# sandialabs/tenzing

Measured on AMD Instinct MI355X. Metric: best-schedule iter time (ms) + MCTS search wall-clock, 3D halo-exchange 8 ranks, lower is better.
Workload: dtype fp64

## Files before the change

### tenzing_amd/csrc/bind/module.cpp

```cpp
#include <pybind11/functional.h>
#include <pybind11/numpy.h>
#include <pybind11/pybind11.h>
#include <pybind11/stl.h>

#include "core/benchmark.hpp"
#include "core/health.hpp"
#include "core/solve.hpp"
#include "hip/comm_ops.hpp"
#include "hip/hip_runtime.hpp"
#include "hip/rccl_comm.hpp"
#include "hip/rocsparse_spmv.hpp"
#include "kernels/kernels.hpp"
#include "workloads/workloads.hpp"

#include <hip/hip_runtime_api.h>

#include <csignal>
#include <cstdlib>
#include <execinfo.h>
#include <sstream>
#include <unistd.h>
#include <vector>

namespace py = pybind11;
// ... 545 lines not shown
        for (auto &x : in) l.append(py::bytes(x));
        return l;
      }, "personalized exchange: element j goes to rank j; returns what each rank sent me");
  py::class_<SelfCtrl, Ctrl, std::shared_ptr<SelfCtrl>>(m, "SelfCtrl").def(py::init<>());
  py::class_<TcpCtrl, Ctrl, std::shared_ptr<TcpCtrl>>(m, "TcpCtrl")
      .def(py::init<int, int>())
      .def("listen", &TcpCtrl::listen, py::arg("port") = 0, py::arg("bind_addr") = "0.0.0.0")
      .def("connect", &TcpCtrl::connect, py::arg("host"), py::arg("port"), py::arg("timeout_s") = 300.0,
           py::call_guard<py::gil_scoped_release>())
      .def("rendezvous", &TcpCtrl::rendezvous, py::arg("host"), py::arg("port"),
           py::arg("timeout_s") = 300.0, py::arg("nports") = 8, py::call_guard<py::gil_scoped_release>(),
           "rank 0 listens on the first free port of port..port+nports-1, the others connect "
           "(handshake-checked): no store, no torch")
      .def("rendezvous_file", &TcpCtrl::rendezvous_file, py::arg("path"), py::arg("host") = "127.0.0.1",
           py::arg("timeout_s") = 300.0, py::call_guard<py::gil_scoped_release>())
      .def("ensure_timeout", &TcpCtrl::ensure_timeout, py::arg("seconds"),
           "raise the peer sockets' receive timeout to at least this (never lowered)")
      .def_property_readonly("timeout", &TcpCtrl::timeout,
                             "the peer sockets' receive timeout in seconds (0 = none)");
  py::class_<MpiCtrl, Ctrl, std::shared_ptr<MpiCtrl>>(m, "MpiCtrl")
      .def(py::init<const std::string &>(), py::arg("lib") = "", py::call_guard<py::gil_scoped_release>())
      .def_static("launched", &MpiCtrl::launched)
      .def_static("launcher_size", &MpiCtrl::launcher_size)
      .def_static("launcher_local_rank", &MpiCtrl::launcher_local_rank)
      .def_property_readonly("library", &MpiCtrl::library);

  py::class_<MctsOpts>(m, "MctsOpts")
      .def(py::init<>())
      .def_readwrite("n_iters", &MctsOpts::n_iters)
      .def_readwrite("time_budget_s", &MctsOpts::time_budget_s)
      .def_readwrite("max_tree_nodes", &MctsOpts::max_tree_nodes)
      .def_readwrite("seed_schedules", &MctsOpts::seed_schedules)
      .def_readwrite("expand_rollout", &MctsOpts::expand_rollout)
      .def_readwrite("remove_redundant_syncs", &MctsOpts::remove_redundant_syncs)
      .def_readwrite("reuse_measurements", &MctsOpts::reuse_measurements)
      .def_readwrite("verify", &MctsOpts::verify)
      .def_readwrite("dump_tree", &MctsOpts::dump_tree)
      .def_readwrite("dump_tree_prefix", &MctsOpts::dump_tree_prefix)
      .def_readwrite("strategy", &MctsOpts::strategy)
      .def_readwrite("seed", &MctsOpts::seed)
      .def_readwrite("explore_c", &MctsOpts::explore_c)
      .def_readwrite("bench", &MctsOpts::bench)
      .def_readwrite("checkpoint_path", &MctsOpts::checkpoint_path)
      .def_readwrite("checkpoint_every", &MctsOpts::checkpoint_every)
      .def_readwrite("resume_path", &MctsOpts::resume_path)
      .def_readwrite("trap_signals", &MctsOpts::trap_signals)
      .def_readwrite("skip_failed", &MctsOpts::skip_failed)
      .def("json", [](const MctsOpts &o) { return o.json().dump(); });
  py::class_<DfsOpts>(m, "DfsOpts")
      .def(py::init<>())
      .def_readwrite("max_seqs", &DfsOpts::max_seqs)
      .def_readwrite("dedup_states", &DfsOpts::dedup_states)
      .def_readwrite("remove_redundant_syncs", &DfsOpts::remove_redundant_syncs)
      .def_readwrite("bench", &DfsOpts::bench)
      .def_readwrite("trap_signals", &DfsOpts::trap_signals)
      .def_readwrite("skip_failed", &DfsOpts::skip_failed)
      .def("json", [](const DfsOpts &o) { return o.json().dump(); });
  py::class_<SimResult>(m, "SimResult")
      .def_readonly("seq", &SimResult::seq)
      .def_readonly("res", &SimResult::res)
      .def_readonly("cached", &SimResult::cached)
      .def_readonly("seeded", &SimResult::seeded);
  py::class_<SearchResult>(m, "SearchResult")
      .def_readonly("sims", &SearchResult::sims)
      .def_readonly("wall_s", &SearchResult::wall_s)
      .def_readonly("tree_size", &SearchResult::tree_size)
      .def_readonly("tree_fully_visited", &SearchResult::tree_fully_visited)
      .def_readonly("stop_reason", &SearchResult::stop_reason)
      .def_readonly("failed", &SearchResult::failed)
      .def_readonly("dead_domains", &SearchResult::dead_domains)
      .def_readonly("pruned_dead", &SearchResult::pruned_dead)
      .def("best", &SearchResult::best)
      .def("counters", [](const SearchResult &r) { return counters_dict(r.counters); })
      .def("counter_counts", [](const SearchResult &r) {
        py::dict d;
        for (const auto &kv : r.counters.counts) d[py::str(kv.first)] = kv.second;
        return d;
      }, "how often each counter was hit (phases; SEED_IN_TREE: seeds placed in the tree)")
      .def("dump_csv", [](const SearchResult &r) {
        std::ostringstream ss;
        r.dump_csv(ss);
        return ss.str();
      })
      .def("dump_jsonl", [](const SearchResult &r) {
        std::ostringstream ss;
        r.dump_jsonl(ss);
        return ss.str();
      });
  py::class_<RunDeadline>(m, "RunDeadline")
      .def(py::init<double, int>(), py::arg("seconds"), py::arg("exit_code") = 5)
      .def("set_report", &RunDeadline::set_report, py::arg("line"))
      .def("cancel", &RunDeadline::cancel)
      .def("tighten", &RunDeadline::tighten, py::arg("seconds"), py::arg("exit_code"),
           "expire at the latest `seconds` from now, exiting with `exit_code`")
      .def_property_readonly("remaining", &RunDeadline::remaining)
      .def_property_readonly("armed", &RunDeadline::armed);
  m.def("exit_with_report", [](int code, const std::string &why) { exit_with_report(code, why); },
        py::arg("code"), py::arg("why"),
        "leave the process now (no cleanup), printing the armed RunDeadline's report line with "
        "\"exit_reason\" added: what the watchdog does when a hung run cannot be released");
  m.def("mcts_explore", [](std::shared_ptr<Graph> g, const Platform &p, Benchmarker &b, Ctrl &c,
                           const MctsOpts &o, py::object cb) {
    std::function<void(size_t, const SimResult &)> f;
    if (!cb.is_none()) {
// ... 437 lines not shown
  py::class_<DistSpmv, std::shared_ptr<DistSpmv>>(m, "DistSpmv")
      .def(py::init([](const SpmvArgs &a, Ctrl *c) {
             py::gil_scoped_release r;
             return std::make_shared<DistSpmv>(a, c);
           }), py::arg("args"), py::arg("ctrl") = nullptr)
      .def_property_readonly("args", &DistSpmv::args)
      .def("local_rows", &DistSpmv::local_rows)
      .def("local_nnz", &DistSpmv::local_nnz)
      .def("remote_nnz", &DistSpmv::remote_nnz)
      .def("remote_cols", &DistSpmv::remote_cols)
      .def("send_elems", &DistSpmv::send_elems)
      .def("num_peers", &DistSpmv::num_peers)
      .def("transport", &DistSpmv::transport)
      .def("uses_ipc", &DistSpmv::uses_ipc)
      .def("uses_rccl", &DistSpmv::uses_rccl)
      .def("rccl_graph_ok", &DistSpmv::rccl_graph_ok, "RCCL exchanges may be captured into hipGraphs")
      .def("rccl_capture_note", &DistSpmv::rccl_capture_note,
           "how the RCCL exchange is compiled into hipGraphs (its preflight's verdict), or why not")
      .def("ipc_errors", &DistSpmv::ipc_errors, py::call_guard<py::gil_scoped_release>())
      .def("setup", [](DistSpmv &s, Ctrl *c) { s.setup(c); }, py::arg("ctrl") = nullptr,
           py::call_guard<py::gil_scoped_release>())
      .def("ready", &DistSpmv::ready)
      .def("add_to_graph", &DistSpmv::add_to_graph)
      .def("op_graph", [](DistSpmv &s) { return std::const_pointer_cast<Graph>(s.op_graph()); })
      .def("check", [](DistSpmv &s, uintptr_t st) { return s.check(P(st)); }, py::arg("stream") = 0)
      .def("reset_y", [](DistSpmv &s, uintptr_t st) { s.reset_y(P(st)); }, py::arg("stream") = 0);
  m.def("move_spmv_op", [](std::shared_ptr<HaloExchange> h, std::vector<int> dirs, std::shared_ptr<DistSpmv> s,
                           std::string name, int lanes, bool intoY) {
    return make_move_spmv_op(h, std::move(dirs), s, std::move(name), lanes, intoY);
  }, py::arg("halo"), py::arg("dirs"), py::arg("spmv"), py::arg("name"), py::arg("lanes") = kern::kSpmvIlp + 4,
     py::arg("into_y") = true,
     "one GPU op running the halo's self moves `dirs` and the SpMV's local product in one kernel "
     "(horizontal fusion; the SpMV's workgroups interleaved among the move's)");
  m.def("random_band_matrix", [](int64_t n, int64_t bw, int64_t nnz, uint64_t seed) {
    CsrHost a = random_band_matrix(n, bw, nnz, seed);
    return py::make_tuple(a.rowPtr, a.colInd, a.val);
  });
  m.def("spd_band_matrix", [](int64_t n, int64_t bw, int64_t nnz, uint64_t seed) {
    CsrHost a = spd_band_matrix(n, bw, nnz, seed);
    return py::make_tuple(a.rowPtr, a.colInd, a.val);
  }, py::arg("n"), py::arg("bw"), py::arg("nnz"), py::arg("seed"),
     "symmetric, strictly diagonally dominant band matrix (mirrored random_band_matrix off-diagonals, "
     "a_ii = 1 + sum |a_ij|) as (rowPtr, colInd, val)");
  py::class_<CgArgs>(m, "CgArgs")
      .def(py::init<>())
      .def_readwrite("m", &CgArgs::m)
      .def_readwrite("bw", &CgArgs::bw)
      .def_readwrite("nnz", &CgArgs::nnz)
      .def_readonly("nnz_actual", &CgArgs::nnz_actual)
      .def_readwrite("seed", &CgArgs::seed)
      .def_readwrite("matrix", &CgArgs::matrix)
      .def_readwrite("device", &CgArgs::device)
      .def_readwrite("form", &CgArgs::form)
      .def_readwrite("lanes", &CgArgs::lanes)
      .def_readwrite("rhs", &CgArgs::rhs)
      .def_readwrite("nrhs", &CgArgs::nrhs)
      .def_readwrite("rhs_first", &CgArgs::rhs_first)
      .def_readwrite("prefix", &CgArgs::prefix)
      .def_readwrite("rank", &CgArgs::rank)
      .def_readwrite("size", &CgArgs::size)
      .def("json", [](const CgArgs &a) { return a.json().dump(); });
  {
    auto f32 = [](const std::vector<float> &v) { return py::array_t<float>(py::ssize_t(v.size()), v.data()); };
    py::class_<ConjugateGradient, std::shared_ptr<ConjugateGradient>>(m, "ConjugateGradient")
        .def(py::init([](const CgArgs &a) { return std::make_shared<ConjugateGradient>(a); }), py::arg("args"))
        .def_property_readonly("args", &ConjugateGradient::args)
// ... 477 lines not shown
```

### tenzing_amd/csrc/core/solve.cpp

```cpp
#include "solve.hpp"
#include "health.hpp"

#include <algorithm>
#include <chrono>
#include <cmath>
#include <condition_variable>
#include <csignal>
#include <cstdio>
#include <cstring>
#include <unistd.h>

#include <atomic>
#include <fstream>
#include <iostream>
#include <limits>
#include <map>
#include <mutex>
#include <sstream>
#include <thread>
#include <unordered_map>
#include <unordered_set>

#ifndef TZ_VERSION_MAJOR
#define TZ_VERSION_MAJOR 0
// ... 230 lines not shown
  void backprop(MctsNode &node, const BenchResult &br) override { push_sorted(node.times, br.pct10); }
};

}

std::vector<std::string> strategy_names() {
  return {"FastMin", "Coverage", "Random", "AvgTime", "Unvisited", "AntiCorrelation",
          "NormalizedAntiCorrelation", "NormRootCorr", "BalanceHistogram"};
}

std::unique_ptr<Strategy> make_strategy(const std::string &name, uint64_t seed) {
  std::string n = name;
  std::transform(n.begin(), n.end(), n.begin(), ::tolower);
  n.erase(std::remove(n.begin(), n.end(), '_'), n.end());
  if (n == "fastmin" || n == "mintime") return std::make_unique<FastMin>();
  if (n == "coverage") return std::make_unique<Coverage>();
  if (n == "random") return std::make_unique<RandomS>(seed);
  if (n == "avgtime") return std::make_unique<AvgTime>();
  if (n == "unvisited") return std::make_unique<Unvisited>();
  if (n == "anticorrelation" || n == "anticorr") return std::make_unique<AntiCorrelation>();
  if (n == "normalizedanticorrelation" || n == "normanticorr") return std::make_unique<NormCorr>(true);
  if (n == "normrootcorr") return std::make_unique<NormCorr>(false);
  if (n == "balancehistogram" || n == "balancehist") return std::make_unique<BalanceHistogram>();
  TZ_THROW("unknown MCTS strategy '" << name << "'");
}


Json MctsOpts::json() const {
  Json j, o;
  o["nIters"] = n_iters;
  o["timeBudgetS"] = time_budget_s;
  if (max_tree_nodes > 0) o["maxTreeNodes"] = max_tree_nodes;
  o["expandRollout"] = expand_rollout;
  o["removeRedundantSyncs"] = remove_redundant_syncs;
  o["reuseMeasurements"] = reuse_measurements;
  o["strategy"] = strategy;
  o["seed"] = int64_t(seed);
  o["exploreC"] = explore_c;
  o["benchOpts"] = bench.json();
  j["mcts__Opts"] = o;
  return j;
}

namespace {

struct Tree {
  MctsNode root;
  std::unique_ptr<Strategy> strat;
  std::mt19937_64 rng;
  double c;
  size_t nodes = 1;
  std::set<std::string> dead;
  size_t prunedDead = 0;

  bool dead_decision(const State &st, const Decision &d) const {
    if (dead.empty()) return false;
    if (d.kind == Decision::Kind::Choose) {
      const auto alts = static_cast<const ChoiceOp &>(*st.graph().op(d.node)).choices();
      return uses_domain(alts[size_t(d.choice)], dead);
    }
    if (d.kind == Decision::Kind::Execute && d.op) return uses_domain(d.op, dead);
    if (d.kind == Decision::Kind::Assign) return uses_domain(st.graph().op(d.node), dead);
    return false;
  }

  static void propagate_visited(MctsNode *node) {
    for (; node; node = node->parent) {
      if (node->children.empty() || node->fully_visited) continue;
      bool all = true;
      for (auto &ch : node->children) all = all && ch->fully_visited;
      if (!all) break;
      node->fully_visited = true;
    }
  }

  bool prune_dead_children(MctsNode &node, const State &st) {
    bool live = false;
    if (!dead.empty())
      for (auto &ch : node.children)
        if (!ch->fully_visited && dead_decision(st, ch->decision)) {
          ch->fully_visited = true;
          ++prunedDead;
        }
    for (auto &ch : node.children) live = live || !ch->fully_visited;
    if (!node.children.empty() && !live) propagate_visited(&node);
    return live || node.children.empty();
// ... 171 lines not shown
        const Decision &d = ch[i]->decision;
        if (d.kind != Decision::Kind::Execute || d.op->op_class() != OpClass::Sync || d.op->kind() != want.kind())
          continue;
        if (ws < 0 || (m != relabel.end() && m->second == sync_stream(*d.op))) pick = int(i);
      }
      ++pos;
      if (pick < 0) continue;
    }
    if (pick < 0 && pos < seed.size()) {
      for (size_t i = 0; i < ch.size() && pick < 0; ++i) {
        const Decision &d = ch[i]->decision;
        if (d.kind == Decision::Kind::Execute && d.op->op_class() != OpClass::Sync &&
            d.op->name() == seed[pos]->name()) {
          pick = int(i);
          advance = true;
        }
      }
    }
    for (size_t i = 0; i < ch.size() && pick < 0; ++i) {
      const Decision &d = ch[i]->decision;
      if (d.kind == Decision::Kind::Execute && d.op->op_class() == OpClass::Sync) pick = int(i);
    }
    if (pick < 0) return nullptr;
    if (advance) ++pos;
    st.apply_inplace(ch[size_t(pick)]->decision);
    cur = ch[size_t(pick)].get();
  }
  tree.ensure_children(*cur, st);
  Sequence s = st.sequence();
  if (removeRedundant) remove_redundant_syncs(s, st.graph(), nStreams);
  return s.canonical_key() == seed.canonical_key() ? cur : nullptr;
}

void graphviz_rec(const MctsNode &node, const Strategy &strat, std::ostream &os, size_t &count,
                  size_t maxNodes, const std::string &id) {
  std::string color = node.fully_visited ? "green" : "black";
  os << "  " << id << " [label=\"" << node.decision.desc() << "\\nn=" << node.n << "\\n"
     << strat.label(node) << "\", color=" << color << "];\n";
  ++count;
  size_t i = 0;
  for (const auto &ch : node.children) {
    ++i;
    if (count >= maxNodes) break;
    if (ch->n == 0) continue;
    const std::string cid = id + "_" + std::to_string(i);
    if (ch->fully_visited || ch->n == 1) {
      os << "  " << cid << " [label=\"" << ch->decision.desc() << "\\nn=" << ch->n
         << "\", color=" << (ch->fully_visited ? "green" : "gray") << "];\n";
      ++count;
    } else {
      graphviz_rec(*ch, strat, os, count, maxNodes, cid);
    }
    os << "  " << id << " -> " << cid << ";\n";
  }
}

void write_file(const std::string &path, const std::string &s) {
  std::ofstream f(path);
  f << s;
}

}

std::string mcts_tree_graphviz(const MctsNode &root, const Strategy &strat, size_t maxNodes) {
  std::ostringstream os;
  os << "digraph MCTS {\n";
// ... 87 lines not shown
      continue;
    }
    Sequence s = root ? opts.seed_schedules[size_t(k)] : index.sequence_from_json(m.at("seq"));
    SimResult sr;
    sr.seq = s;
    sr.seeded = true;
    try {
      ScopedTimer t(result.counters, "BENCHMARK");
      sr.res = bench.benchmark(s, opts.bench);
    } catch (const std::exception &e) {
      if (!opts.skip_failed || !skippable(e, ctrl)) throw;
      if (root) {
        ++result.failed;
        TZ_LOG(Warn, "seed schedule " << k << " skipped: " << e.what());
      }
      after_failure();
      continue;
    }
    if (root) {
      cache.emplace(s.canonical_key(), result.sims.size());
      if (opts.remove_redundant_syncs) {
        try {
          Sequence r = s;
          if (remove_redundant_syncs(r, *resolve_graph(*gp, s), plat.n_streams) > 0)
            cache.emplace(r.canonical_key(), result.sims.size());
        } catch (const std::exception &) {
        }
      }
      result.sims.push_back(sr);
      if (onResult) onResult(result.sims.size() - 1, sr);
      MctsNode *leaf = seed_path(tree, rootState, s, opts.remove_redundant_syncs, plat.n_streams);
      if (leaf) {
        tree.backprop(leaf, sr.res);
        result.counters.add("SEED_IN_TREE", 0.0);
      }
      TZ_LOG(Info, "seed schedule " << k << " pct10=" << sr.res.pct10
                                    << (leaf ? " (in the tree)" : " (no tree path)"));
    }
  }

  std::function<void(int)> dump = [&result](int) { result.dump_csv(std::cout); };
  if (root && opts.trap_signals) register_handler(dump);

  auto checkpoint = [&]() {
    if (!root || opts.checkpoint_path.empty()) return;
    Json ck;
    ck["tree"] = tree.save(tree.root);
    Json sims = Json::array();
    for (const auto &s : result.sims) {
      Json j;
      j["result"] = s.res.json();
      j["seq"] = s.seq.json();
      if (s.seeded) j["seeded"] = true;
      sims.push_back(j);
    }
    ck["sims"] = sims;
    ck["opts"] = opts.json();
    write_file(opts.checkpoint_path + ".tmp", ck.dump());
    std::rename((opts.checkpoint_path + ".tmp").c_str(), opts.checkpoint_path.c_str());
  };

  Counters &C = result.counters;
  for (int64_t iter = 0;; ++iter) {
    int64_t stop = 0;
    if (root) {
      if (tree.root.fully_visited) {
        stop = 1;
        result.stop_reason = "full_tree";
      } else if (opts.n_iters > 0 && iter >= opts.n_iters) {
        stop = 2;
        result.stop_reason = "iterations";
      } else if (opts.time_budget_s > 0 && wtime() - t0 > opts.time_budget_s) {
        stop = 3;
        result.stop_reason = "time_budget";
      } else if (opts.max_tree_nodes > 0 && tree.nodes >= size_t(opts.max_tree_nodes)) {
        stop = 5;
        result.stop_reason = "large_tree";
      }
      if (opts.trap_signals && signal_pending()) {
        stop = 4;
        result.stop_reason = "signal";
      }
    }
    stop = ctrl.bcast_int(stop, 0);
    if (stop == 4) {
      ctrl.barrier();
      if (root) handle_pending_signal();
      std::exit(1);
    }
    if (stop) break;

    std::string msg;
    MctsNode *bpStart = nullptr;
    size_t cachedIdx = size_t(-1);
    Sequence seq;
    if (root) {
      bool found = false;
      for (int attempt = 0; attempt < 64 && !found && !tree.root.fully_visited; ++attempt) {
        State st = rootState;
        MctsNode *node = &tree.root;
        bool dead = false;
        {
          ScopedTimer t(C, "SELECT");
          while (!node->is_leaf() && !node->terminal) {
            if (!tree.prune_dead_children(*node, st)) {
              dead = true;
              break;
            }
            node = tree.pick_uct(*node);
            st.apply_inplace(node->decision);
          }
        }
        if (dead) continue;
        {
          ScopedTimer t(C, "EXPAND");
          tree.ensure_children(*node, st);
          if (!node->children.empty()) {
            if (!tree.prune_dead_children(*node, st)) continue;
            MctsNode *next = nullptr;
            for (auto &ch : node->children)
              if (ch->n == 0 && !ch->fully_visited) {
                next = ch.get();
                break;
              }
            if (!next) next = tree.pick_uct(*node);
            node = next;
            st.apply_inplace(node->decision);
          }
        }
        {
          ScopedTimer t(C, "ROLLOUT");
          bpStart = node;
          MctsNode *cur = node;
          std::vector<size_t> live;
          while (!st.complete() && !dead) {
            if (opts.expand_rollout) {
              tree.ensure_children(*cur, st);
              TZ_CHECK(!cur->children.empty(), "dead-end state during rollout");
              live.clear();
              for (size_t i = 0; i < cur->children.size(); ++i)
                if (!tree.dead_decision(st, cur->children[i]->decision)) live.push_back(i);
              if (live.empty()) {
                tree.prune_dead_children(*cur, st);
                dead = true;
                break;
              }
              std::uniform_int_distribution<size_t> u(0, live.size() - 1);
              cur = cur->children[live[u(tree.rng)]].get();
              st.apply_inplace(cur->decision);
              bpStart = cur;
            } else {
              auto ds = st.get_decisions();
              TZ_CHECK(!ds.empty(), "dead-end state during rollout");
              live.clear();
              for (size_t i = 0; i < ds.size(); ++i)
                if (!tree.dead_decision(st, ds[i])) live.push_back(i);
              if (live.empty()) {
                dead = true;
                break;
              }
              std::uniform_int_distribution<size_t> u(0, live.size() - 1);
              st.apply_inplace(ds[live[u(tree.rng)]]);
            }
          }
          if (dead) continue;
          if (opts.expand_rollout) tree.ensure_children(*cur, st);
        }
// ... 39 lines not shown
        try {
          br = bench.benchmark(seq, opts.bench);
        } catch (const std::exception &e) {
          if (!skippable(e, ctrl)) throw;
          failed = true;
          if (root) TZ_LOG(Warn, "mcts iter " << iter << ": candidate skipped: " << e.what());
        }
      } else {
        br = bench.benchmark(seq, opts.bench);
      }
    }
    if (failed) {
      if (root) {
        ++result.failed;
        tree.prune_failed(bpStart);
      }
      after_failure();
      continue;
    }
    if (root) {
      SimResult sr;
      sr.seq = seq;
      if (cached) {
        sr.res = result.sims[cachedIdx].res;
        sr.cached = true;
      } else {
        sr.res = br;
        cache.emplace(seq.canonical_key(), result.sims.size());
      }
      result.sims.push_back(sr);
      {
        ScopedTimer t(C, "BACKPROP");
        tree.backprop(bpStart, sr.res);
      }
      if (onResult) onResult(result.sims.size() - 1, sr);
      TZ_LOG(Info, "mcts iter " << iter << " pct10=" << sr.res.pct10 << (cached ? " (cached)" : "")
                                << " tree=" << tree.root.size());
      if (opts.dump_tree && (iter < 10 || (iter < 50 && iter % 10 == 0) ||
                             (iter < 100 && iter % 25 == 0))) {
        write_file(opts.dump_tree_prefix + std::to_string(iter) + ".dot",
                   mcts_tree_graphviz(tree.root, *tree.strat));
      }
      if (opts.checkpoint_every > 0 && (iter + 1) % opts.checkpoint_every == 0) checkpoint();
    }
  }
  ctrl.barrier();
  if (root) {
    unregister_handler();
    checkpoint();
    result.tree_size = tree.root.size();
    result.tree_fully_visited = tree.root.fully_visited_size();
  }
  result.dead_domains.assign(tree.dead.begin(), tree.dead.end());
  result.pruned_dead = tree.prunedDead;
  result.wall_s = wtime() - t0;
  return result;
}


Json DfsOpts::json() const {
  Json j, o;
  o["maxSeqs"] = max_seqs;
  j["dfs__Opts"] = o;
  return j;
}

std::vector<Sequence> get_all_sequences(const Graph &g, const Platform &plat, int64_t maxSeqs,
                                        bool dedupStates, bool removeRedundant) {
  auto gp = std::make_shared<Graph>(g);
  gp->normalize();
  std::vector<State> work{State(gp, plat)};
  std::unordered_set<std::string> seenStates, seenSeqs;
  std::vector<Sequence> out;
  while (!work.empty()) {
    if (maxSeqs >= 0 && int64_t(out.size()) >= maxSeqs) break;
    State cur = std::move(work.back());
    work.pop_back();
    if (cur.complete()) {
      Sequence s = cur.sequence();
      if (removeRedundant) remove_redundant_syncs(s, cur.graph(), plat.n_streams);
      if (seenSeqs.insert(s.canonical_key()).second) out.push_back(std::move(s));
      continue;
    }
    auto ds = cur.get_decisions();
// ... 282 lines not shown
```

### tenzing_amd/csrc/core/solve.hpp

```cpp
#pragma once

#include "benchmark.hpp"
#include "util.hpp"

#include <functional>
#include <limits>
#include <memory>
#include <ostream>
#include <random>

namespace tz {

struct SimResult {
  Sequence seq;
  BenchResult res;
  bool cached = false;
  bool seeded = false;
};

struct SearchResult {
  std::vector<SimResult> sims;
  Counters counters;
  Json opts;
  double wall_s = 0;
  size_t tree_size = 0;
  size_t tree_fully_visited = 0;
  std::string stop_reason;
  size_t failed = 0;
  std::vector<std::string> dead_domains;
  size_t pruned_dead = 0;

  int best() const;
  void dump_csv(std::ostream &os) const;
  void dump_jsonl(std::ostream &os) const;
};


struct MctsNode {
  MctsNode *parent = nullptr;
  std::vector<std::unique_ptr<MctsNode>> children;
  Decision decision;
  bool expanded = false;
  bool fully_visited = false;
  bool terminal = false;
  size_t n = 0;
  double tmin = std::numeric_limits<double>::infinity();
  double tmax = -std::numeric_limits<double>::infinity();
  std::vector<double> times;

  const MctsNode &root() const { return parent ? parent->root() : *this; }
  size_t size() const;
  size_t fully_visited_size() const;
  size_t unvisited_size() const;
  bool is_leaf() const;
};

class Strategy {
public:
  virtual ~Strategy() = default;
  virtual std::string name() const = 0;
  virtual double select(const MctsNode &child) = 0;
  virtual void backprop(MctsNode &node, const BenchResult &br) = 0;
  virtual std::string label(const MctsNode &node) const;
};

std::unique_ptr<Strategy> make_strategy(const std::string &name, uint64_t seed);
std::vector<std::string> strategy_names();

struct MctsOpts {
  int64_t n_iters = 300;
  double time_budget_s = 0;
  int64_t max_tree_nodes = 0;
  bool expand_rollout = true;
  bool remove_redundant_syncs = true;
  bool reuse_measurements = true;
  bool verify = true;
  bool skip_failed = true;
  bool dump_tree = false;
  std::string dump_tree_prefix = "mcts_";
  std::string strategy = "FastMin";
  uint64_t seed = 0;
  double explore_c = 1.41421356;
  BenchOpts bench;
  std::string checkpoint_path;
  int64_t checkpoint_every = 0;
  bool trap_signals = false;
  std::string resume_path;
  std::vector<Sequence> seed_schedules;
  Json json() const;
};

SearchResult mcts_explore(const Graph &g, const Platform &plat, Benchmarker &bench, Ctrl &ctrl,
                          const MctsOpts &opts,
                          const std::function<void(size_t, const SimResult &)> &onResult = nullptr);

std::string mcts_tree_graphviz(const MctsNode &root, const Strategy &strat, size_t maxNodes = 2000);


struct DfsOpts {
  int64_t max_seqs = -1;
  bool dedup_states = true;
  bool remove_redundant_syncs = true;
  bool trap_signals = false;
  bool skip_failed = true;
  BenchOpts bench;
  Json json() const;
};

std::vector<Sequence> get_all_sequences(const Graph &g, const Platform &plat, int64_t maxSeqs = -1,
                                        bool dedupStates = true, bool removeRedundant = true);

SearchResult dfs_explore(const Graph &g, const Platform &plat, Benchmarker &bench, Ctrl &ctrl,
                         const DfsOpts &opts,
                         const std::function<void(size_t, const SimResult &)> &onResult = nullptr);


void register_handler(std::function<void(int)> fn);
void unregister_handler();
int signal_pending();
[[noreturn]] void handle_pending_signal();

class RunDeadline {
public:
// ... 23 lines not shown
```

### tenzing_amd/csrc/core/state.cpp

```cpp
#include "state.hpp"
#include "util.hpp"

#include <algorithm>
#include <map>
#include <sstream>
#include <unordered_map>

namespace tz {


Json Sequence::json(bool inGraph) const {
  Json a = Json::array();
  for (const auto &e : entries) {
    Json j = e.op->json();
    if (inGraph) j["in_graph"] = e.op->op_class() != OpClass::Sync;
    a.push_back(j);
  }
  return a;
}

std::string Sequence::desc(const std::string &delim) const {
  std::string s;
  for (size_t i = 0; i < entries.size(); ++i) {
    if (i) s += delim;
// ... 538 lines not shown
    for (int i = int(seq.size()) - 1; i >= 0; --i) {
      if (skip[i] || seq.entries[i].op->op_class() != OpClass::Sync) continue;
      skip[i] = 1;
      if (check(seq, g, nStreams, true, &skip).empty()) {
        ++removed;
        changed = true;
      } else {
        skip[i] = 0;
      }
    }
  }
  if (removed) {
    Sequence out;
    for (size_t i = 0; i < seq.size(); ++i)
      if (!skip[i]) out.entries.push_back(seq.entries[i]);
    seq = std::move(out);
  }
  return removed;
}

namespace {
bool runs_any(const OpPtr &op, const std::set<std::string> &names) {
  if (names.count(op->name())) return true;
  if (op->op_class() == OpClass::Compound) {
    const auto &sub = *static_cast<const CompoundOp &>(*op).graph();
    for (int v : sub.vertices())
      if (v != Graph::kStart && v != Graph::kFinish && runs_any(sub.op(v), names)) return true;
  } else if (op->op_class() == OpClass::Choice) {
    for (const auto &alt : static_cast<const ChoiceOp &>(*op).choices())
      if (runs_any(alt, names)) return true;
  }
  return false;
}
}

GraphPtr resolve_graph(const Graph &g, const Sequence &seq) {
  std::set<std::string> names;
  for (const auto &e : seq.entries) {
    const OpClass c = e.op->op_class();
    if (c == OpClass::BoundGpu)
      names.insert(static_cast<const BoundGpuOp &>(*e.op).unbound()->name());
    else if (c != OpClass::Sync)
      names.insert(e.op->name());
  }
  auto cur = std::make_shared<Graph>(g);
  for (bool changed = true; changed;) {
    changed = false;
    for (int v : cur->vertices()) {
      const OpPtr op = cur->op(v);
      if (op->op_class() == OpClass::Compound) {
        cur = cur->clone_but_expand(v, *static_cast<const CompoundOp &>(*op).graph());
        changed = true;
        break;
      }
      if (op->op_class() == OpClass::Choice) {
        OpPtr pick;
        for (const auto &alt : static_cast<const ChoiceOp &>(*op).choices()) {
          if (!runs_any(alt, names)) continue;
          TZ_CHECK(!pick, "sequence runs two alternatives of " << op->name() << ": "
                                                               << pick->name() << ", " << alt->name());
          pick = alt;
        }
        TZ_CHECK(pick, "sequence runs no alternative of " << op->name());
        cur = cur->clone_but_replace(v, pick);
        changed = true;
        break;
      }
    }
  }
  return cur;
}

Sequence random_rollout(State s, std::mt19937_64 &rng) {
  while (!s.complete()) {
    auto ds = s.get_decisions();
    TZ_CHECK(!ds.empty(), "dead end state (no decisions, not complete)");
    std::uniform_int_distribution<size_t> u(0, ds.size() - 1);
    s.apply_inplace(ds[u(rng)]);
  }
  return s.sequence();
}

}
```

### tenzing_amd/csrc/core/state.hpp

```cpp
#pragma once

#include "graph.hpp"

#include <algorithm>
#include <random>
#include <set>
#include <string>
#include <vector>

namespace tz {

struct Platform {
  int n_streams = 2;
  bool symmetric_streams = true;
  bool offer_stream_sync = false;

  static Platform make_n_streams(int n) {
    Platform p;
    p.n_streams = n;
    return p;
  }
};

struct SeqEntry {
// ... 87 lines not shown
  int domain_pred(const BoundOp &op) const;

private:
  BoundOpPtr bound_op(int node) const;
  void grow();
  std::vector<int> used_streams() const;
  std::vector<int> all_preds(int node, const BoundOp &op) const;

  GraphPtr g_;
  Platform plat_;
  Sequence seq_;
  std::vector<int> streamOf_;
  std::vector<int> posOf_;
  std::vector<int> stamp_;
  SyncModel sync_;
  std::set<std::string> transforms_;
  std::vector<std::pair<std::string, int>> domainLast_;
};

bool equivalent(const State &a, const State &b);


struct Violation {
  int position;
  std::string op;
  std::string pred;
  std::string desc() const;
};

std::vector<Violation> verify(const Sequence &seq, const Graph &g, int nStreams);

GraphPtr resolve_graph(const Graph &g, const Sequence &seq);

int remove_redundant_syncs(Sequence &seq, const Graph &g, int nStreams);

Sequence random_rollout(State s, std::mt19937_64 &rng);

}
```

### tenzing_amd/csrc/workloads/fused_ops.cpp

```cpp
#include "workloads.hpp"

#include "core/util.hpp"

#include <algorithm>

namespace tz {

namespace {

class MoveSpmv : public GpuOp {
public:
  MoveSpmv(std::shared_ptr<const HaloExchange> h, std::vector<int> dirs, std::shared_ptr<const DistSpmv> s,
           std::string name, int lanes, bool intoY)
      : h_(std::move(h)), dirs_(std::move(dirs)), s_(std::move(s)), name_(std::move(name)), lanes_(lanes),
        intoY_(intoY) {
    TZ_CHECK(lanes_ > kern::kSpmvIlp && lanes_ <= kern::kSpmvIlp + 4 && (lanes_ - kern::kSpmvIlp) != 3,
             name_ << ": lanes must be kSpmvIlp + 1, 2 or 4");
    for (int i : dirs_) TZ_CHECK(h_->is_direct(i), name_ << ": direction " << i << " is not a self move");
    TZ_CHECK(int(dirs_.size()) <= kern::kMaxBoxes, name_ << ": at most " << kern::kMaxBoxes << " directions");
  }
  std::string name() const override { return name_; }
  std::string kind() const override { return "MoveSpmv"; }
  double move_bytes() const {
    double b = 0;
    for (int i : dirs_) b += 2.0 * 8.0 * double(h_->box_elems(i));
    return b;
  }
  double spmv_bytes() const { return 12.0 * double(s_->local_nnz()) + 8.0 * double(s_->local_rows()); }
  double cost_us() const override {
    const double mv = 3.0 + move_bytes() / 5.0e6, sp = 4.0 + spmv_bytes() / 3.0e6;
    return std::max(mv, sp) + 0.5 * std::min(mv, sp);
  }
  std::vector<Traffic> traffic() const override { return {{"hbm", "kernel", move_bytes() + spmv_bytes()}}; }
  double latency_us() const override { return 3.0; }
  void launch(void *s, Executor &) const override {
    const std::vector<kern::MoveDesc> ms = h_->direct_moves(dirs_);
    TZ_CHECK(int(ms.size()) <= kern::kMaxBoxes, name_ << ": too many moves for one launch");
    kern::box_move_spmv(ms.data(), int(ms.size()), s_->local_job(lanes_, intoY_), s);
  }

private:
  std::shared_ptr<const HaloExchange> h_;
  std::vector<int> dirs_;
  std::shared_ptr<const DistSpmv> s_;
  std::string name_;
  int lanes_;
  bool intoY_;
};

}

std::shared_ptr<GpuOp> make_move_spmv_op(std::shared_ptr<const HaloExchange> h, std::vector<int> dirs,
                                         std::shared_ptr<const DistSpmv> s, std::string name, int lanes,
                                         bool intoY) {
  return std::make_shared<MoveSpmv>(std::move(h), std::move(dirs), std::move(s), std::move(name), lanes, intoY);
}

}
```

### tenzing_amd/csrc/workloads/workloads.hpp

```cpp
#pragma once

#include "core/ctrl.hpp"
#include "core/graph.hpp"
#include "kernels/kernels.hpp"

#include <algorithm>
#include <array>
#include <functional>
#include <map>
#include <memory>
#include <mutex>
#include <string>
#include <vector>

namespace tz {

class RcclComm;
class RocsparseCsr;

double preflight_limit_s(double dflt);

class LoweredLimit {
public:
  LoweredLimit(double &v, double limit) : v_(v), keep_(v) { v_ = std::min(v_, limit); }
// ... 556 lines not shown

private:
  std::vector<float> down(const DeviceBuffer &d, int col) const;
  int checked(int col) const;
  std::shared_ptr<Graph> form_graph(bool fused) const;
  std::shared_ptr<Graph> sr_graph() const;
  CgArgs a_;
  CsrHost A_;
  std::vector<std::vector<float>> b_;
  DeviceBuffer dRow_, dCol_, dVal_, dB_, dX_, dR_, dP_, dQ_;
  DeviceBuffer dS_, dW_;
  DeviceBuffer dScal_;
  double *pq_() const { return dScal_.as<double>(); }
  double *rrp_() const { return dScal_.as<double>() + kern::kCgMaxPartials; }
  double *rr_() const { return dScal_.as<double>() + 2 * kern::kCgMaxPartials; }
  double *alpha_() const { return rr_() + 1; }
  double *beta_() const { return rr_() + 2; }
  double *srGamma_() const { return rr_() + 3; }
  double *srAlpha_() const { return rr_() + 4; }
  double *srBeta_() const { return rr_() + 5; }
  double *srGammaPrev_() const { return rr_() + 6; }
  double *srAlphaPrev_() const { return rr_() + 7; }
  double *scratch_() const { return rr_() + 8; }
  DeviceBuffer dBatch_;
  double *bDelta_() const { return dBatch_.as<double>(); }
  double *bGamma_() const { return bDelta_() + a_.nrhs * kern::kCgMaxPartials; }
  double *bScal_(int i) const { return bGamma_() + a_.nrhs * kern::kCgMaxPartials + i * a_.nrhs; }
};

std::shared_ptr<GpuOp> make_move_spmv_op(std::shared_ptr<const HaloExchange> h, std::vector<int> dirs,
                                         std::shared_ptr<const DistSpmv> s, std::string name, int lanes,
                                         bool into_y);

}
```

### tenzing_amd/models/fused.py

```python
from __future__ import annotations

import dataclasses

from .. import _tz
from .halo import HaloConfig, build_halo
from .spmv import SpmvConfig, build_spmv

SPMV_ILP = 1000


def build_fused(halo_cfg: HaloConfig, spmv_cfg: SpmvConfig, ctrl=None, device: int = -1,
                setup: bool = True, horizontal: bool = True):
    g = _tz.Graph()
    h, _ = build_halo(halo_cfg, ctrl, device, setup, g)
    sp = dataclasses.replace(spmv_cfg, prefix=spmv_cfg.prefix or "spmv_")
    s, _ = build_spmv(sp, ctrl, device, setup, g)
    size = ctrl.size if ctrl is not None else 1
    direct = [i for i in range(h.ndirs()) if h.is_direct(i)]
    if horizontal and size == 1 and len(direct) == h.ndirs() and not halo_cfg.stencil:
        alts = [_tz.StaticCompoundOp("hs_separate", g)]
        for w in (4, 2):
            alts.append(_tz.move_spmv_op(h, direct, s, f"hs_onelaunch_i{w}", SPMV_ILP + w, True))
        top = _tz.StaticChoiceOp("hs_launches", alts)
        g = _tz.Graph()
        g.start_then(top)
        g.then_finish(top)
    return h, s, g
```

Measured before the change: 0.04458.

## Guide MCTS choice rollouts by best schedule and add serial fused alternative

Adds a guide_choices MCTS mode, on by default. The first unvisited ChoiceOp alternatives are rolled out by copying the best known schedule's op order, stream assignment and sub-choices, and near the end of the search each top-level alternative is closed over with such a guided rollout. The fused graph construction moves into C++ and gains a serial alternative (halo then SpMV), plus an hs_order choice on one rank. The aim is a fairer comparison between coarse alternatives without spending many random rollouts, at the cost of extra bookkeeping and a larger search space.

```diff
diff --git a/tenzing_amd/csrc/bind/module.cpp b/tenzing_amd/csrc/bind/module.cpp
--- a/tenzing_amd/csrc/bind/module.cpp
+++ b/tenzing_amd/csrc/bind/module.cpp
@@ -601,6 +601,7 @@
       .def_readwrite("max_tree_nodes", &MctsOpts::max_tree_nodes)
       .def_readwrite("seed_schedules", &MctsOpts::seed_schedules)
       .def_readwrite("expand_rollout", &MctsOpts::expand_rollout)
+      .def_readwrite("guide_choices", &MctsOpts::guide_choices)
       .def_readwrite("remove_redundant_syncs", &MctsOpts::remove_redundant_syncs)
       .def_readwrite("reuse_measurements", &MctsOpts::reuse_measurements)
       .def_readwrite("verify", &MctsOpts::verify)
@@ -639,6 +640,7 @@
       .def_readonly("failed", &SearchResult::failed)
       .def_readonly("dead_domains", &SearchResult::dead_domains)
       .def_readonly("pruned_dead", &SearchResult::pruned_dead)
+      .def_readonly("top_choice_visits", &SearchResult::top_choice_visits)
       .def("best", &SearchResult::best)
       .def("counters", [](const SearchResult &r) { return counters_dict(r.counters); })
       .def("counter_counts", [](const SearchResult &r) {
@@ -1142,6 +1144,11 @@
      py::arg("into_y") = true,
      "one GPU op running the halo's self moves `dirs` and the SpMV's local product in one kernel "
      "(horizontal fusion; the SpMV's workgroups interleaved among the move's)");
+  m.def("fused_graph", [](std::shared_ptr<HaloExchange> h, std::shared_ptr<DistSpmv> s, bool horizontal) {
+    return fused_graph(h, s, horizontal);
+  }, py::arg("halo"), py::arg("spmv"), py::arg("horizontal") = true,
+     "BASELINE config 5's graph: both workloads' ops; with `horizontal` under the top-level ChoiceOp "
+     "hs_launches (hs_separate, hs_serial, and on one rank hs_onelaunch_i4 / _i2)");
   m.def("random_band_matrix", [](int64_t n, int64_t bw, int64_t nnz, uint64_t seed) {
     CsrHost a = random_band_matrix(n, bw, nnz, seed);
     return py::make_tuple(a.rowPtr, a.colInd, a.val);
diff --git a/tenzing_amd/csrc/core/solve.cpp b/tenzing_amd/csrc/core/solve.cpp
--- a/tenzing_amd/csrc/core/solve.cpp
+++ b/tenzing_amd/csrc/core/solve.cpp
@@ -286,6 +286,7 @@
   o["timeBudgetS"] = time_budget_s;
   if (max_tree_nodes > 0) o["maxTreeNodes"] = max_tree_nodes;
   o["expandRollout"] = expand_rollout;
+  o["guideChoices"] = guide_choices;
   o["removeRedundantSyncs"] = remove_redundant_syncs;
   o["reuseMeasurements"] = reuse_measurements;
   o["strategy"] = strategy;
@@ -306,6 +307,21 @@
   size_t nodes = 1;
   std::set<std::string> dead;
   size_t prunedDead = 0;
+  std::unordered_map<const MctsNode *, std::pair<double, size_t>> bestBelow;
+
+  void note_result(const MctsNode *leaf, double pct10, size_t sim) {
+    for (const MctsNode *n = leaf; n; n = n->parent) {
+      auto it = bestBelow.find(n);
+      if (it == bestBelow.end() || pct10 < it->second.first) bestBelow[n] = {pct10, sim};
+    }
+  }
+  int best_near(const MctsNode *n) const {
+    for (n = n ? n->parent : nullptr; n; n = n->parent) {
+      auto it = bestBelow.find(n);
+      if (it != bestBelow.end()) return int(it->second.second);
+    }
+    return -1;
+  }
 
   bool dead_decision(const State &st, const Decision &d) const {
     if (dead.empty()) return false;
@@ -543,6 +559,152 @@
   return s.canonical_key() == seed.canonical_key() ? cur : nullptr;
 }
 
+struct Guide {
+  std::set<std::string> names;
+  std::unordered_map<std::string, int> streamOf;
+  std::unordered_map<std::string, size_t> posOf;
+  std::unordered_map<int, int> relabel;
+
+  std::vector<std::string> taken;
+
+  Guide(const Sequence &s, const Graph &g) {
+    for (size_t i = 0; i < s.size(); ++i) {
+      const BoundOp &op = *s[i];
+      const OpClass c = op.op_class();
+      if (c == OpClass::Sync || c == OpClass::Start || c == OpClass::Finish) continue;
+      names.insert(op.name());
+      posOf.emplace(op.name(), i);
+      if (c == OpClass::BoundGpu) streamOf[op.name()] = static_cast<const BoundGpuOp &>(op).stream();
+    }
+    std::set<const Graph *> seen;
+    collect_taken(g, seen);
+  }
+
+  void collect_taken(const OpPtr &op, std::set<const Graph *> &seen) {
+    if (op->op_class() == OpClass::Compound) {
+      collect_taken(*static_cast<const CompoundOp &>(*op).graph(), seen);
+    } else if (op->op_class() == OpClass::Choice) {
+      const auto &choice = static_cast<const ChoiceOp &>(*op);
+      const int k = alternative(choice);
+      const auto alts = choice.choices();
+      if (k >= 0) taken.push_back(alts[size_t(k)]->name());
+      for (const auto &a : alts) collect_taken(a, seen);
+    }
+  }
+  void collect_taken(const Graph &g, std::set<const Graph *> &seen) {
+    if (!seen.insert(&g).second) return;
+    for (int v : g.vertices()) collect_taken(g.op(v), seen);
+  }
+
+  int alternative(const ChoiceOp &choice) const {
+    try {
+      return alternative_of(choice, names);
+    } catch (const std::exception &) {
+      return -1;
+    }
+  }
+
+  int by_analogy(const ChoiceOp &choice) const {
+    const auto alts = choice.choices();
+    int best = 0;
+    size_t bestLen = 3;
+    for (size_t i = 0; i < alts.size(); ++i) {
+      const std::string a = alts[i]->name();
+      for (const std::string &t : taken) {
+        size_t l = 0;
+        while (l < a.size() && l < t.size() && a[a.size() - 1 - l] == t[t.size() - 1 - l]) ++l;
+        if (l > bestLen) {
+          bestLen = l;
+          best = int(i);
+        }
+      }
+    }
+    return best;
+  }
+
+  int pick(const State &st, const std::vector<Decision> &ds, const std::function<bool(const Decision &)> &live) {
+    using K = Decision::Kind;
+    auto first_of = [&](K k) {
+      for (size_t i = 0; i < ds.size(); ++i)
+        if (ds[i].kind == k && live(ds[i])) return int(i);
+      return -1;
+    };
+    int p = first_of(K::Expand);
+    if (p >= 0) return p;
+    if ((p = first_of(K::Choose)) >= 0) {
+      const int v = ds[size_t(p)].node;
+      const auto &choice = static_cast<const ChoiceOp &>(*st.graph().op(v));
+      int want = alternative(choice);
+      if (want < 0) want = by_analogy(choice);
+      for (size_t i = 0; i < ds.size(); ++i)
+        if (ds[i].kind == K::Choose && ds[i].node == v && ds[i].choice == want && live(ds[i]))
+          return int(i);
+      return p;
+    }
+    if ((p = first_of(K::Assign)) >= 0) {
+      const int v = ds[size_t(p)].node;
+      auto offered = [&](int s) {
+        for (size_t i = 0; i < ds.size(); ++i)
+          if (ds[i].kind == K::Assign && ds[i].node == v && ds[i].stream == s && live(ds[i])) return int(i);
+        return -1;
+      };
+      auto it = streamOf.find(st.graph().op(v)->name());
+      if (it == streamOf.end()) return p;
+      auto m = relabel.find(it->second);
+      if (m != relabel.end()) return std::max(offered(m->second), p);
+      for (size_t i = 0; i < ds.size(); ++i) {
+        if (ds[i].kind != K::Assign || ds[i].node != v || !live(ds[i])) continue;
+        bool taken = false;
+        for (const auto &kv : relabel) taken = taken || kv.second == ds[i].stream;
+        if (taken) continue;
+        relabel[it->second] = ds[i].stream;
+        return int(i);
+      }
+      return p;
+    }
+    int best = -1, sync = -1;
+    size_t bestPos = 0;
+    for (size_t i = 0; i < ds.size(); ++i) {
+      if (ds[i].kind != K::Execute || !live(ds[i])) continue;
+      if (ds[i].node < 0) {
+        if (sync < 0) sync = int(i);
+        continue;
+      }
+      auto it = posOf.find(ds[i].op->name());
+      const size_t pos = it == posOf.end() ? size_t(-1) : it->second;
+      if (best < 0 || pos < bestPos) {
+        best = int(i);
+        bestPos = pos;
+      }
+    }
+    return best >= 0 ? best : sync;
+  }
+};
+
+bool guided_rollout(Tree &tree, State &st, MctsNode **cur, Guide guide) {
+  const std::function<bool(const Decision &)> live = [&](const Decision &d) { return !tree.dead_decision(st, d); };
+  std::vector<Decision> ds;
+  while (!st.complete()) {
+    if (cur) {
+      tree.ensure_children(**cur, st);
+      ds.clear();
+      for (const auto &ch : (*cur)->children) ds.push_back(ch->decision);
+    } else {
+      ds = st.get_decisions();
+    }
+    TZ_CHECK(!ds.empty(), "dead-end state during rollout");
+    const int p = guide.pick(st, ds, live);
+    if (p < 0) {
+      if (cur) tree.prune_dead_children(**cur, st);
+      return false;
+    }
+    if (cur) *cur = (*cur)->children[size_t(p)].get();
+    st.apply_inplace(ds[size_t(p)]);
+  }
+  if (cur) tree.ensure_children(**cur, st);
+  return true;
+}
+
 void graphviz_rec(const MctsNode &node, const Strategy &strat, std::ostream &os, size_t &count,
                   size_t maxNodes, const std::string &id) {
   std::string color = node.fully_visited ? "green" : "black";
@@ -696,6 +858,7 @@
       MctsNode *leaf = seed_path(tree, rootState, s, opts.remove_redundant_syncs, plat.n_streams);
       if (leaf) {
         tree.backprop(leaf, sr.res);
+        tree.note_result(leaf, sr.res.pct10, result.sims.size() - 1);
         result.counters.add("SEED_IN_TREE", 0.0);
       }
       TZ_LOG(Info, "seed schedule " << k << " pct10=" << sr.res.pct10
@@ -725,16 +888,77 @@
   };
 
   Counters &C = result.counters;
+  MctsNode *topNode = nullptr;
+  State topState = rootState;
+  if (root && opts.guide_choices) {
+    MctsNode *node = &tree.root;
+    while (!topState.complete()) {
+      tree.ensure_children(*node, topState);
+      const auto &ch = node->children;
+      if (ch.size() == 1 && ch[0]->decision.kind != Decision::Kind::Choose) {
+        node = ch[0].get();
+        topState.apply_inplace(node->decision);
+        continue;
+      }
+      bool one = ch.size() >= 2 && ch.size() <= size_t(kFewAlternatives);
+      for (const auto &c : ch)
+        one = one && c->decision.kind == Decision::Kind::Choose && c->decision.node == ch[0]->decision.node;
+      if (one) topNode = node;
+      break;
+    }
+  }
+  const int64_t nTop = topNode ? int64_t(topNode->children.size()) : 0;
+  std::vector<size_t> closing;
+  bool closed = false;
+
+  std::string msg;
+  MctsNode *bpStart = nullptr;
+  size_t cachedIdx = size_t(-1);
+  Sequence seq;
+  auto close_over = [&](size_t k) {
+    const int b = result.best();
+    if (b < 0) return false;
+    State st = topState;
+    MctsNode *cur = topNode->children[k].get();
+    if (cur->fully_visited || tree.dead_decision(st, cur->decision)) return false;
+    st.apply_inplace(cur->decision);
+    bpStart = cur;
+    if (!guided_rollout(tree, st, opts.expand_rollout ? &cur : nullptr, Guide(result.sims[size_t(b)].seq, *gp)))
+      return false;
+    if (opts.expand_rollout) bpStart = cur;
+    seq = st.sequence();
+    if (opts.remove_redundant_syncs) remove_redundant_syncs(seq, st.graph(), plat.n_streams);
+    if (cache.count(seq.canonical_key())) return false;
+    if (opts.verify) {
+      auto v = verify(seq, st.graph(), plat.n_streams);
+      if (!v.empty()) TZ_THROW("candidate schedule has a race: " << v[0].desc());
+    }
+    return true;
+  };
+
   for (int64_t iter = 0;; ++iter) {
     int64_t stop = 0;
+    bool found = false;
     if (root) {
-      if (tree.root.fully_visited) {
+      const bool timeUp = opts.time_budget_s > 0 && wtime() - t0 > opts.time_budget_s;
+      if (nTop > 0 && !closed && (timeUp || (opts.n_iters >= 4 * nTop && iter >= opts.n_iters - nTop))) {
+        closed = true;
+        for (size_t k = 0; k < size_t(nTop); ++k) closing.push_back(k);
+      }
+      if (!(opts.n_iters > 0 && iter >= opts.n_iters))
+        while (!closing.empty() && !found) {
+          const size_t k = closing.back();
+          closing.pop_back();
+          found = close_over(k);
+        }
+      if (found) {
+      } else if (tree.root.fully_visited) {
         stop = 1;
         result.stop_reason = "full_tree";
       } else if (opts.n_iters > 0 && iter >= opts.n_iters) {
         stop = 2;
         result.stop_reason = "iterations";
-      } else if (opts.time_budget_s > 0 && wtime() - t0 > opts.time_budget_s) {
+      } else if (timeUp) {
         stop = 3;
         result.stop_reason = "time_budget";
       } else if (opts.max_tree_nodes > 0 && tree.nodes >= size_t(opts.max_tree_nodes)) {
@@ -754,12 +978,9 @@
     }
     if (stop) break;
 
-    std::string msg;
-    MctsNode *bpStart = nullptr;
-    size_t cachedIdx = size_t(-1);
-    Sequence seq;
+    msg.clear();
+    cachedIdx = size_t(-1);
     if (root) {
-      bool found = false;
       for (int attempt = 0; attempt < 64 && !found && !tree.root.fully_visited; ++attempt) {
         State st = rootState;
         MctsNode *node = &tree.root;
@@ -782,11 +1003,13 @@
           if (!node->children.empty()) {
             if (!tree.prune_dead_children(*node, st)) continue;
             MctsNode *next = nullptr;
-            for (auto &ch : node->children)
-              if (ch->n == 0 && !ch->fully_visited) {
-                next = ch.get();
-                break;
-              }
+            for (int pass = opts.guide_choices ? 0 : 1; pass < 2 && !next; ++pass)
+              for (auto &ch : node->children)
+                if (ch->n == 0 && !ch->fully_visited &&
+                    (pass == 1 || ch->decision.kind == Decision::Kind::Choose)) {
+                  next = ch.get();
+                  break;
+                }
             if (!next) next = tree.pick_uct(*node);
             node = next;
             st.apply_inplace(node->decision);
@@ -797,6 +1020,14 @@
           bpStart = node;
           MctsNode *cur = node;
           std::vector<size_t> live;
+          const int guide = opts.guide_choices && node->n == 0 && node->decision.kind == Decision::Kind::Choose
+                                ? tree.best_near(node)
+                                : -1;
+          if (guide >= 0) {
+            dead = !guided_rollout(tree, st, opts.expand_rollout ? &cur : nullptr,
+                                   Guide(result.sims[size_t(guide)].seq, *gp));
+            if (opts.expand_rollout) bpStart = cur;
+          }
           while (!st.complete() && !dead) {
             if (opts.expand_rollout) {
               tree.ensure_children(*cur, st);
@@ -902,6 +1133,7 @@
       {
         ScopedTimer t(C, "BACKPROP");
         tree.backprop(bpStart, sr.res);
+        tree.note_result(bpStart, sr.res.pct10, result.sims.size() - 1);
       }
       if (onResult) onResult(result.sims.size() - 1, sr);
       TZ_LOG(Info, "mcts iter " << iter << " pct10=" << sr.res.pct10 << (cached ? " (cached)" : "")
@@ -920,6 +1152,11 @@
     checkpoint();
     result.tree_size = tree.root.size();
     result.tree_fully_visited = tree.root.fully_visited_size();
+    if (topNode) {
+      const auto alts = static_cast<const ChoiceOp &>(*topState.graph().op(topNode->children[0]->decision.node)).choices();
+      for (const auto &ch : topNode->children)
+        result.top_choice_visits.emplace_back(alts[size_t(ch->decision.choice)]->name(), ch->n);
+    }
   }
   result.dead_domains.assign(tree.dead.begin(), tree.dead.end());
   result.pruned_dead = tree.prunedDead;
diff --git a/tenzing_amd/csrc/core/solve.hpp b/tenzing_amd/csrc/core/solve.hpp
--- a/tenzing_amd/csrc/core/solve.hpp
+++ b/tenzing_amd/csrc/core/solve.hpp
@@ -29,6 +29,7 @@
   size_t failed = 0;
   std::vector<std::string> dead_domains;
   size_t pruned_dead = 0;
+  std::vector<std::pair<std::string, size_t>> top_choice_visits;
 
   int best() const;
   void dump_csv(std::ostream &os) const;
@@ -72,6 +73,7 @@
   double time_budget_s = 0;
   int64_t max_tree_nodes = 0;
   bool expand_rollout = true;
+  bool guide_choices = true;
   bool remove_redundant_syncs = true;
   bool reuse_measurements = true;
   bool verify = true;
@@ -89,6 +91,8 @@
   std::vector<Sequence> seed_schedules;
   Json json() const;
 };
+
+constexpr int kFewAlternatives = 8;
 
 SearchResult mcts_explore(const Graph &g, const Platform &plat, Benchmarker &bench, Ctrl &ctrl,
                           const MctsOpts &opts,
diff --git a/tenzing_amd/csrc/core/state.cpp b/tenzing_amd/csrc/core/state.cpp
--- a/tenzing_amd/csrc/core/state.cpp
+++ b/tenzing_amd/csrc/core/state.cpp
@@ -594,6 +594,36 @@
   }
   return false;
 }
+void runs_which(const OpPtr &op, const std::set<std::string> &names, std::set<std::string> &out) {
+  if (names.count(op->name())) out.insert(op->name());
+  if (op->op_class() == OpClass::Compound) {
+    const auto &sub = *static_cast<const CompoundOp &>(*op).graph();
+    for (int v : sub.vertices())
+      if (v != Graph::kStart && v != Graph::kFinish) runs_which(sub.op(v), names, out);
+  } else if (op->op_class() == OpClass::Choice) {
+    for (const auto &alt : static_cast<const ChoiceOp &>(*op).choices()) runs_which(alt, names, out);
+  }
+}
+}
+
+int alternative_of(const ChoiceOp &choice, const std::set<std::string> &names) {
+  const auto alts = choice.choices();
+  int pick = -1;
+  std::set<std::string> got;
+  std::vector<std::set<std::string>> all(alts.size());
+  for (size_t i = 0; i < alts.size(); ++i) {
+    if (!runs_any(alts[i], names)) continue;
+    runs_which(alts[i], names, all[i]);
+    if (pick < 0 || all[i].size() > got.size()) {
+      pick = int(i);
+      got = all[i];
+    }
+  }
+  for (size_t i = 0; i < alts.size() && pick >= 0; ++i)
+    TZ_CHECK(std::includes(got.begin(), got.end(), all[i].begin(), all[i].end()),
+             "sequence runs two alternatives of " << choice.name() << ": " << alts[size_t(pick)]->name()
+                                                  << ", " << alts[i]->name());
+  return pick;
 }
 
 GraphPtr resolve_graph(const Graph &g, const Sequence &seq) {
@@ -616,15 +646,10 @@
         break;
       }
       if (op->op_class() == OpClass::Choice) {
-        OpPtr pick;
-        for (const auto &alt : static_cast<const ChoiceOp &>(*op).choices()) {
-          if (!runs_any(alt, names)) continue;
-          TZ_CHECK(!pick, "sequence runs two alternatives of " << op->name() << ": "
-                                                               << pick->name() << ", " << alt->name());
-          pick = alt;
-        }
-        TZ_CHECK(pick, "sequence runs no alternative of " << op->name());
-        cur = cur->clone_but_replace(v, pick);
+        const auto &choice = static_cast<const ChoiceOp &>(*op);
+        const int pick = alternative_of(choice, names);
+        TZ_CHECK(pick >= 0, "sequence runs no alternative of " << op->name());
+        cur = cur->clone_but_replace(v, choice.choices()[size_t(pick)]);
         changed = true;
         break;
       }
diff --git a/tenzing_amd/csrc/core/state.hpp b/tenzing_amd/csrc/core/state.hpp
--- a/tenzing_amd/csrc/core/state.hpp
+++ b/tenzing_amd/csrc/core/state.hpp
@@ -143,6 +143,8 @@
 
 GraphPtr resolve_graph(const Graph &g, const Sequence &seq);
 
+int alternative_of(const ChoiceOp &choice, const std::set<std::string> &names);
+
 int remove_redundant_syncs(Sequence &seq, const Graph &g, int nStreams);
 
 Sequence random_rollout(State s, std::mt19937_64 &rng);
diff --git a/tenzing_amd/csrc/workloads/fused_ops.cpp b/tenzing_amd/csrc/workloads/fused_ops.cpp
--- a/tenzing_amd/csrc/workloads/fused_ops.cpp
+++ b/tenzing_amd/csrc/workloads/fused_ops.cpp
@@ -56,4 +56,42 @@
   return std::make_shared<MoveSpmv>(std::move(h), std::move(dirs), std::move(s), std::move(name), lanes, intoY);
 }
 
+std::shared_ptr<Graph> fused_graph(const std::shared_ptr<HaloExchange> &h, const std::shared_ptr<DistSpmv> &s,
+                                   bool horizontal) {
+  auto both = std::make_shared<Graph>();
+  h->add_to_graph(*both);
+  s->add_to_graph(*both);
+  if (!horizontal || h->args().stencil) return both;
+  auto gh = std::make_shared<Graph>(), gs = std::make_shared<Graph>(), ser = std::make_shared<Graph>();
+  h->add_to_graph(*gh);
+  s->add_to_graph(*gs);
+  auto ch = std::make_shared<StaticCompoundOp>("hs_serial_halo", gh);
+  auto cs = std::make_shared<StaticCompoundOp>("hs_serial_spmv", gs);
+  ser->start_then(ch);
+  ser->then(ch, cs);
+  ser->then_finish(cs);
+  auto serial = std::make_shared<StaticCompoundOp>("hs_serial", ser);
+  std::vector<int> direct;
+  for (int i = 0; i < h->ndirs(); ++i)
+    if (h->is_direct(i)) direct.push_back(i);
+  std::vector<OpPtr> alts;
+  if (h->args().size == 1 && int(direct.size()) == h->ndirs()) {
+    auto sep = std::make_shared<Graph>();
+    auto order = std::make_shared<StaticChoiceOp>(
+        "hs_order", std::vector<OpPtr>{std::make_shared<StaticCompoundOp>("hs_forked", both), serial});
+    sep->start_then(order);
+    sep->then_finish(order);
+    alts.push_back(std::make_shared<StaticCompoundOp>("hs_separate", sep));
+    for (int w : {4, 2})
+      alts.push_back(make_move_spmv_op(h, direct, s, "hs_onelaunch_i" + std::to_string(w), kern::kSpmvIlp + w, true));
+  } else {
+    alts = {std::make_shared<StaticCompoundOp>("hs_separate", both), serial};
+  }
+  auto top = std::make_shared<StaticChoiceOp>("hs_launches", alts);
+  auto g = std::make_shared<Graph>();
+  g->start_then(top);
+  g->then_finish(top);
+  return g;
 }
+
+}
diff --git a/tenzing_amd/csrc/workloads/workloads.hpp b/tenzing_amd/csrc/workloads/workloads.hpp
--- a/tenzing_amd/csrc/workloads/workloads.hpp
+++ b/tenzing_amd/csrc/workloads/workloads.hpp
@@ -612,4 +612,7 @@
                                          std::shared_ptr<const DistSpmv> s, std::string name, int lanes,
                                          bool into_y);
 
+std::shared_ptr<Graph> fused_graph(const std::shared_ptr<HaloExchange> &h, const std::shared_ptr<DistSpmv> &s,
+                                   bool horizontal);
+
 }
diff --git a/tenzing_amd/models/fused.py b/tenzing_amd/models/fused.py
--- a/tenzing_amd/models/fused.py
+++ b/tenzing_amd/models/fused.py
@@ -3,26 +3,19 @@
 import dataclasses
 
 from .. import _tz
-from .halo import HaloConfig, build_halo
-from .spmv import SpmvConfig, build_spmv
-
-SPMV_ILP = 1000
+from .halo import HaloConfig
+from .spmv import SpmvConfig
 
 
 def build_fused(halo_cfg: HaloConfig, spmv_cfg: SpmvConfig, ctrl=None, device: int = -1,
                 setup: bool = True, horizontal: bool = True):
-    g = _tz.Graph()
-    h, _ = build_halo(halo_cfg, ctrl, device, setup, g)
+    rank = ctrl.rank if ctrl is not None else 0
+    size = ctrl.size if ctrl is not None else 1
+    h = _tz.HaloExchange(halo_cfg.args(rank, size, device))
+    if setup:
+        h.setup(ctrl)
     sp = dataclasses.replace(spmv_cfg, prefix=spmv_cfg.prefix or "spmv_")
-    s, _ = build_spmv(sp, ctrl, device, setup, g)
-    size = ctrl.size if ctrl is not None else 1
-    direct = [i for i in range(h.ndirs()) if h.is_direct(i)]
-    if horizontal and size == 1 and len(direct) == h.ndirs() and not halo_cfg.stencil:
-        alts = [_tz.StaticCompoundOp("hs_separate", g)]
-        for w in (4, 2):
-            alts.append(_tz.move_spmv_op(h, direct, s, f"hs_onelaunch_i{w}", SPMV_ILP + w, True))
-        top = _tz.StaticChoiceOp("hs_launches", alts)
-        g = _tz.Graph()
-        g.start_then(top)
-        g.then_finish(top)
-    return h, s, g
+    s = _tz.DistSpmv(sp.args(rank, size, device), ctrl if size > 1 else None)
+    if setup:
+        s.setup(ctrl)
+    return h, s, _tz.fused_graph(h, s, horizontal)
```

New measurement: 0.04457 (median of 3 runs). About the same (-0.0%).
